# atakan-topaloglu/stable-virtual-camera

Hardware: AMD Instinct MI355X
Metric: denoising steps/sec, 1.3B Seva @ 21x576x576 views (higher is better)
Workload: dtype f16; 1 GPU; Seva 1.3B (1,263,968,004 params, random-init), one 21-view window per GPU, 576x576 px (latent 72x72), CFG batch 42, Euler-EDM step, MultiviewCFG(1.2) cfg 2.0; novel_views_per_sec = value x (T - 1 input view) / 50 steps per window; views=21, latent=72, windows=1

## Files before the change

### stable-virtual-camera_amd/csrc/attention.hip

```cpp
#include "attn_common.h"

#include <stdlib.h>

namespace {
typedef __fp16 p16x2_t __attribute__((ext_vector_type(2)));
__device__ __forceinline__ p16x2_t pack_p(float e0, float e1) {
  return __builtin_bit_cast(p16x2_t, __builtin_convertvector(f32x2{e0, e1}, half2_t));
}

struct AttnArgs : AttnBase {};

typedef short short8_t __attribute__((ext_vector_type(8)));

__device__ __forceinline__ half8_t tr_read_pair(const char* a0, const char* a1) {
  short4_t lo = __builtin_amdgcn_ds_read_tr16_b64_v4i16((__attribute__((address_space(3))) short4_t*)a0);
  short4_t hi = __builtin_amdgcn_ds_read_tr16_b64_v4i16((__attribute__((address_space(3))) short4_t*)a1);
  short8_t s = __builtin_shufflevector(lo, hi, 0, 1, 2, 3, 4, 5, 6, 7);
  return __builtin_bit_cast(half8_t, s);
}

__device__ __forceinline__ int v_chunk_swz(int row, int chunk) { return chunk ^ (((row >> 1) & 1) << 2); }

__device__ __forceinline__ float half_wave_max(float v) {
  float a = v, b = v;
  asm volatile("s_nop 1\n\tv_permlane32_swap_b32 %0, %1" : "+v"(a), "+v"(b));
  return fmaxf(a, b);
}

template <int NW, int KT, bool USE_TR, bool DBGK, bool PRE, int NBUF = 3>
__global__ __launch_bounds__(NW * 64, 3) void attn_kernel(AttnArgs p) {
  constexpr int KB = KT / 32;
  const int dbg = DBGK ? p.dbg : 0;
  static_assert(NBUF == 3 || NBUF == 1, "the three-buffer ring, or one buffer for a single tile");
  static_assert(NBUF * 2 * KT * 128 >= NW * 32 * 128, "the epilogue stages NW images of 32 rows in the K/V buffers");

  __shared__ __attribute__((aligned(16))) char smem[NBUF * 2 * KT * 128];
  constexpr int BUF_BYTES = 2 * KT * 128;
  typedef AttnRing<KT, NW, BUF_BYTES, v_chunk_swz> Ring;

  const int tid = threadIdx.x;
  const int lane = tid & 63;
  const int wave = tid >> 6;
  const int qi = lane & 31, hh = lane >> 5;

  AttnWg w;
  attn_decode<false>(p, KT, w);
  const int qb = w.qb;
  const half_t* const qbase = attn_q_base(p, w);
  const half_t* const kbase = attn_kv_base(p, w, p.k);
  const half_t* const vbase = attn_kv_base(p, w, p.v);
  half_t* const obase = attn_o_base(p, w);

  const int qrow = qb * (32 * NW) + wave * 32 + qi;
  const int qrow_c = qrow < p.lq ? qrow : p.lq - 1;

  half8_t qf[4];
#pragma unroll
  for (int s = 0; s < 4; ++s)
    qf[s] = *(const half8_t*)(qbase + (int64_t)qrow_c * p.q_sl + 16 * s + 8 * hh);

  f32x16 acc_o[2];
#pragma unroll
  for (int d = 0; d < 2; ++d)
#pragma unroll
    for (int r = 0; r < 16; ++r) acc_o[d][r] = 0.f;
  constexpr float RESCALE_THR = 8.0f;
  float m_run = PRE ? 0.f : -1e30f, l_run = 0.f;
  f32x16 neg_m[2];
#pragma unroll
  for (int r = 0; r < 16; ++r) neg_m[0][r] = neg_m[1][r] = 0.f;
  const float c = p.scale_log2;

  const int nt = (p.lk + KT - 1) / KT;
  Ring ring(kbase, vbase, p.k_sl, p.lk, smem, lane, wave);

  const int g16 = lane >> 4, i16 = lane & 15, q4 = i16 >> 2, p4 = i16 & 3;

  auto tile = [&](int buf, auto masked_c, int kt) {
    constexpr bool MASKED = decltype(masked_c)::value;
    const char* const lds_k = smem + buf * BUF_BYTES;
    const char* const lds_v = lds_k + KT * 128;
    const bool more2 = attn_ring_prefetch(kt, nt, buf, !(dbg & 1), ring);

    f32x16 sc[KB];
    __builtin_amdgcn_s_setprio(1);
#pragma unroll
    for (int kb = 0; kb < KB; ++kb) {
      const int krow = 32 * kb + qi;
      if (!(dbg & 8)) {
#pragma unroll
        for (int s = 0; s < 4; ++s) {
          const half8_t kf =
              *(const half8_t*)(lds_k + krow * 128 + (k_chunk_swz(krow, 2 * s + hh) << 4));
          if (s == 0) {
            f32x16 c0;
            if (PRE) {
              c0 = neg_m[kb & 1];
            } else {
#pragma unroll
              for (int r = 0; r < 16; ++r) c0[r] = 0.f;
            }
            sc[kb] = __builtin_amdgcn_mfma_f32_32x32x16_f16(kf, qf[s], c0, 0, 0, 0);
          } else {
            sc[kb] = __builtin_amdgcn_mfma_f32_32x32x16_f16(kf, qf[s], sc[kb], 0, 0, 0);
          }
        }
      } else {
        asm volatile("" : "=v"(sc[kb]));
      }
    }
    __builtin_amdgcn_s_setprio(0);
    if (MASKED) {
#pragma unroll
      for (int kb = 0; kb < KB; ++kb)
#pragma unroll
        for (int r = 0; r < 16; ++r) {
          const int key = kt * KT + 32 * kb + (r & 3) + 8 * (r >> 2) + 4 * hh;
          if (key >= p.lk) sc[kb][r] = -1e30f;
        }
    }
    float mx = -1e30f;
    if (!(dbg & 2)) {
      float mk[KB];
#pragma unroll
      for (int kb = 0; kb < KB; ++kb) {
        mk[kb] = sc[kb][0];
#pragma unroll
        for (int r = 1; r < 16; ++r) mk[kb] = fmaxf(mk[kb], sc[kb][r]);
      }
#pragma unroll
      for (int kb = 0; kb < KB; ++kb) mx = fmaxf(mx, mk[kb]);
      mx = half_wave_max(mx);
    }
    if (PRE) {
      const bool first = kt == 0;
      if (!(dbg & 2) && (first || __any(mx > RESCALE_THR))) {
        const float delta = first ? mx : fmaxf(mx, 0.f);
        const float alpha = first ? 1.0f : __builtin_amdgcn_exp2f(-delta);
        m_run += delta;
#pragma unroll
        for (int r = 0; r < 16; ++r) neg_m[0][r] = neg_m[1][r] = -m_run;
        asm volatile("" : "+v"(neg_m[0]), "+v"(neg_m[1]));
        l_run *= alpha;
#pragma unroll
        for (int d = 0; d < 2; ++d)
#pragma unroll
          for (int r = 0; r < 16; ++r) acc_o[d][r] *= alpha;
#pragma unroll
        for (int kb = 0; kb < KB; ++kb)
#pragma unroll
          for (int r = 0; r < 16; ++r) sc[kb][r] -= delta;
      }
    } else {
    const float mxs = mx * c;
    if (!(dbg & 2) && __any(mxs > m_run + RESCALE_THR)) {
      const float m_new = fmaxf(m_run, mxs);
      const float alpha = __builtin_amdgcn_exp2f(m_run - m_new);
      m_run = m_new;
      l_run *= alpha;
#pragma unroll
      for (int d = 0; d < 2; ++d)
#pragma unroll
        for (int r = 0; r < 16; ++r) acc_o[d][r] *= alpha;
    }
    }
    typedef __fp16 fp16x2_t __attribute__((ext_vector_type(2)));
    const fp16x2_t ones2 = {(__fp16)1.0f, (__fp16)1.0f};
    float lsum4[4] = {0.f, 0.f, 0.f, 0.f};
    half8_t pf[KB][2];
#pragma unroll
    for (int kb = 0; kb < KB; ++kb)
#pragma unroll
      for (int s2 = 0; s2 < 2; ++s2) {
        fp16x2_t pk[4];
#pragma unroll
        for (int j = 0; j < 4; ++j) {
          float e0, e1;
          if (!(dbg & 2)) {
            if (PRE) {
              e0 = __builtin_amdgcn_exp2f(sc[kb][8 * s2 + 2 * j]);
              e1 = __builtin_amdgcn_exp2f(sc[kb][8 * s2 + 2 * j + 1]);
            } else {
              e0 = __builtin_amdgcn_exp2f(__builtin_fmaf(sc[kb][8 * s2 + 2 * j], c, -m_run));
              e1 = __builtin_amdgcn_exp2f(__builtin_fmaf(sc[kb][8 * s2 + 2 * j + 1], c, -m_run));
            }
          } else {
            e0 = sc[kb][8 * s2 + 2 * j];
            e1 = sc[kb][8 * s2 + 2 * j + 1];
          }
          pk[j] = pack_p(e0, e1);
          if (!(dbg & 2)) lsum4[j] = __builtin_amdgcn_fdot2(pk[j], ones2, lsum4[j], false);
        }
        pf[kb][s2] = __builtin_bit_cast(half8_t, pk);
      }
    l_run += (lsum4[0] + lsum4[1]) + (lsum4[2] + lsum4[3]);

    __builtin_amdgcn_s_setprio(1);
#pragma unroll
    for (int db = 0; db < 2; ++db) {
#pragma unroll
      for (int kb = 0; kb < KB; ++kb) {
#pragma unroll
        for (int s2 = 0; s2 < 2; ++s2) {
          const int r0 = 32 * kb + 16 * s2 + 4 * hh;
          half8_t vf;
          if (USE_TR) {
            const int colbyte = (32 * db + 16 * (g16 & 1) + 4 * p4) * 2;
            const int ch = colbyte >> 4, within = colbyte & 15;
            const int ra = r0 + q4, rb = r0 + 8 + q4;
            vf = tr_read_pair(lds_v + ra * 128 + (v_chunk_swz(ra, ch) << 4) + within,
                              lds_v + rb * 128 + (v_chunk_swz(rb, ch) << 4) + within);
          } else {
            const int d = 32 * db + qi;
#pragma unroll
            for (int j = 0; j < 8; ++j) {
              const int row = r0 + (j & 3) + 8 * (j >> 2);
              vf[j] = *(const half_t*)(lds_v + row * 128 + (v_chunk_swz(row, d >> 3) << 4) + (d & 7) * 2);
            }
          }
          if (!(dbg & 4)) acc_o[db] = __builtin_amdgcn_mfma_f32_32x32x16_f16(vf, pf[kb][s2], acc_o[db], 0, 0, 0);
          else asm volatile("" ::"v"(vf), "v"(pf[kb][s2]));
        }
      }
    }
    __builtin_amdgcn_s_setprio(0);
    attn_ring_arrive<Ring::G>(more2);
  };
  attn_ring_start<Ring::G>(nt, ring, qf);
  const int nfull = p.lk / KT;
  int buf = 0;
  for (int kt = 0; kt < nfull; ++kt) {
    tile(buf, std::false_type{}, kt);
    buf = buf == 2 ? 0 : buf + 1;
  }
  if (nfull < nt) tile(buf, std::true_type{}, nfull);

  const float l_tot = l_run + __shfl_xor(l_run, 32, 64);
  const float inv = 1.0f / l_tot;
  __syncthreads();
  char* const ow = smem + wave * (32 * 128);
  attn_stage_o32(ow, qi, hh, acc_o, inv);
  attn_store_rows<4>(ow, obase, p.o_sl, qb * (32 * NW) + wave * 32, p.lq, lane);
}

template <int KT, bool SPLIT = false>
__global__ __launch_bounds__(256, 2) void attn2_kernel(AttnArgs p) {
  constexpr int NW = 4, QB = 2, KB = KT / 32;
  __shared__ __attribute__((aligned(16))) char smem[3 * 2 * KT * 128];
  constexpr int BUF_BYTES = 2 * KT * 128;
  typedef AttnRing<KT, NW, BUF_BYTES, v_chunk_swz> Ring;

  const int tid = threadIdx.x;
  const int lane = tid & 63;
  const int wave = tid >> 6;
  const int qi = lane & 31, hh = lane >> 5;

  AttnWg w;
  attn_decode<SPLIT>(p, KT, w);
  const int qb = w.qb, lk = w.lk;
  const half_t* const qbase = attn_q_base(p, w);
  const half_t* const kbase = attn_kv_base(p, w, p.k);
  const half_t* const vbase = attn_kv_base(p, w, p.v);
  half_t* const obase = attn_o_base(p, w);

  half8_t qf[QB][4];
#pragma unroll
  for (int c = 0; c < QB; ++c) {
    const int qrow = qb * (32 * QB * NW) + wave * (32 * QB) + 32 * c + qi;
    const int qrow_c = qrow < p.lq ? qrow : p.lq - 1;
#pragma unroll
    for (int s = 0; s < 4; ++s)
      qf[c][s] = *(const half8_t*)(qbase + (int64_t)qrow_c * p.q_sl + 16 * s + 8 * hh);
  }

  const bool active = __builtin_amdgcn_readfirstlane(qb * (32 * QB * NW) + wave * (32 * QB)) < p.lq;
  f32x16 acc_o[QB][2];
  float m_run[QB], l_run[QB];
  f32x16 neg_m[QB];
#pragma unroll
  for (int c = 0; c < QB; ++c) {
    m_run[c] = 0.f;
    l_run[c] = 0.f;
#pragma unroll
    for (int r = 0; r < 16; ++r) neg_m[c][r] = 0.f;
#pragma unroll
    for (int d = 0; d < 2; ++d)
#pragma unroll
      for (int r = 0; r < 16; ++r) acc_o[c][d][r] = 0.f;
  }
  constexpr float P_SUM_BOUND = 16384.0f;

  const int nt = (lk + KT - 1) / KT;
  Ring ring(kbase, vbase, p.k_sl, lk, smem, lane, wave);
  const int g16 = lane >> 4, i16 = lane & 15, q4 = i16 >> 2, p4 = i16 & 3;
  typedef __fp16 fp16x2_t __attribute__((ext_vector_type(2)));
  const fp16x2_t ones2 = {(__fp16)1.0f, (__fp16)1.0f};

  auto tile = [&](int buf, auto masked_c, int kt) {
    constexpr bool MASKED = decltype(masked_c)::value;
    const char* const lds_k = smem + buf * BUF_BYTES;
    const char* const lds_v = lds_k + KT * 128;
    const bool more2 = attn_ring_prefetch(kt, nt, buf, true, ring);

    if (active) {
    f32x16 sc[QB][KB];
    __builtin_amdgcn_s_setprio(1);
    if constexpr (!SPLIT) {
      half8_t kfa[KB][4];
#pragma unroll
      for (int kb = 0; kb < KB; ++kb) {
        const int krow = 32 * kb + qi;
#pragma unroll
        for (int s = 0; s < 4; ++s) kfa[kb][s] = *(const half8_t*)(lds_k + krow * 128 + (k_chunk_swz(krow, 2 * s + hh) << 4));
      }
      __builtin_amdgcn_sched_barrier(0);
#pragma unroll
      for (int kb = 0; kb < KB; ++kb)
#pragma unroll
        for (int s = 0; s < 4; ++s)
#pragma unroll
          for (int c = 0; c < QB; ++c)
            sc[c][kb] = __builtin_amdgcn_mfma_f32_32x32x16_f16(kfa[kb][s], qf[c][s], s == 0 ? neg_m[c] : sc[c][kb], 0, 0, 0);
    } else {
#pragma unroll
    for (int kb = 0; kb < KB; ++kb) {
      const int krow = 32 * kb + qi;
#pragma unroll
      for (int s = 0; s < 4; ++s) {
        const half8_t kf = *(const half8_t*)(lds_k + krow * 128 + (k_chunk_swz(krow, 2 * s + hh) << 4));
#pragma unroll
        for (int c = 0; c < QB; ++c) {
          if (s == 0) {
            sc[c][kb] = __builtin_amdgcn_mfma_f32_32x32x16_f16(kf, qf[c][s], neg_m[c], 0, 0, 0);
          } else {
            sc[c][kb] = __builtin_amdgcn_mfma_f32_32x32x16_f16(kf, qf[c][s], sc[c][kb], 0, 0, 0);
          }
        }
      }
    }
    }
    __builtin_amdgcn_s_setprio(0);
    half8_t pf[QB][KB][2];
#pragma unroll
    for (int c = 0; c < QB; ++c) {
      if (MASKED) {
#pragma unroll
        for (int kb = 0; kb < KB; ++kb)
#pragma unroll
          for (int r = 0; r < 16; ++r) {
            const int key = kt * KT + 32 * kb + (r & 3) + 8 * (r >> 2) + 4 * hh;
            if (key >= lk) sc[c][kb][r] = -1e30f;
          }
      }
      float ls[4];
      const auto exp_pack = [&]() {
        ls[0] = ls[1] = ls[2] = ls[3] = 0.f;
#pragma unroll
        for (int kb = 0; kb < KB; ++kb)
#pragma unroll
          for (int s2 = 0; s2 < 2; ++s2) {
            fp16x2_t pk[4];
#pragma unroll
            for (int j = 0; j < 4; ++j) {
              const float e0 = __builtin_amdgcn_exp2f(sc[c][kb][8 * s2 + 2 * j]);
              const float e1 = __builtin_amdgcn_exp2f(sc[c][kb][8 * s2 + 2 * j + 1]);
              pk[j] = pack_p(e0, e1);
              ls[j] = __builtin_amdgcn_fdot2(pk[j], ones2, ls[j], false);
            }
            pf[c][kb][s2] = __builtin_bit_cast(half8_t, pk);
          }
        return (ls[0] + ls[1]) + (ls[2] + ls[3]);
      };
      float tot = exp_pack();
      const bool first = kt == 0;
      if (__builtin_expect(first || __any(!(tot < P_SUM_BOUND)), 0)) {
        float mk[KB];
#pragma unroll
        for (int kb = 0; kb < KB; ++kb) {
          mk[kb] = sc[c][kb][0];
#pragma unroll
          for (int r = 1; r < 16; ++r) mk[kb] = fmaxf(mk[kb], sc[c][kb][r]);
        }
        float mx = mk[0];
#pragma unroll
        for (int kb = 1; kb < KB; ++kb) mx = fmaxf(mx, mk[kb]);
        mx = half_wave_max(mx);
        const float delta = first ? mx : fmaxf(mx, 0.f);
        const float alpha = first ? 1.0f : __builtin_amdgcn_exp2f(-delta);
        m_run[c] += delta;
        l_run[c] *= alpha;
#pragma unroll
        for (int r = 0; r < 16; ++r) neg_m[c][r] = -m_run[c];
#pragma unroll
        for (int d = 0; d < 2; ++d)
#pragma unroll
          for (int r = 0; r < 16; ++r) acc_o[c][d][r] *= alpha;
#pragma unroll
        for (int kb = 0; kb < KB; ++kb)
#pragma unroll
          for (int r = 0; r < 16; ++r) sc[c][kb][r] -= delta;
        tot = exp_pack();
      }
      l_run[c] += tot;
    }
    __builtin_amdgcn_s_setprio(1);
#pragma unroll
    for (int db = 0; db < 2; ++db)
#pragma unroll
      for (int kb = 0; kb < KB; ++kb)
#pragma unroll
        for (int s2 = 0; s2 < 2; ++s2) {
          const int r0 = 32 * kb + 16 * s2 + 4 * hh;
          const int colbyte = (32 * db + 16 * (g16 & 1) + 4 * p4) * 2;
          const int ch = colbyte >> 4, within = colbyte & 15;
          const int ra = r0 + q4, rb = r0 + 8 + q4;
          const half8_t vf = tr_read_pair(lds_v + ra * 128 + (v_chunk_swz(ra, ch) << 4) + within,
                                          lds_v + rb * 128 + (v_chunk_swz(rb, ch) << 4) + within);
#pragma unroll
          for (int c = 0; c < QB; ++c)
            acc_o[c][db] = __builtin_amdgcn_mfma_f32_32x32x16_f16(vf, pf[c][kb][s2], acc_o[c][db], 0, 0, 0);
        }
    __builtin_amdgcn_s_setprio(0);
    }
    attn_ring_arrive<Ring::G>(more2);
  };
  attn_ring_start<Ring::G>(nt, ring, qf);
  const int nfull = lk / KT;
  int buf = 0;
  for (int kt = 0; kt < nfull; ++kt) {
    tile(buf, std::false_type{}, kt);
    buf = buf == 2 ? 0 : buf + 1;
  }
  if (nfull < nt) tile(buf, std::true_type{}, nfull);

  if constexpr (SPLIT) {
    const int64_t row0 = attn_part_row0(p, w);
#pragma unroll
    for (int c = 0; c < QB; ++c) {
      const int qrow = qb * (32 * QB * NW) + wave * (32 * QB) + 32 * c + qi;
      const float l_tot = l_run[c] + __shfl_xor(l_run[c], 32, 64);
      if (qrow < p.lq) {
        float* const po = p.part_o + (row0 + qrow) * 64;
#pragma unroll
        for (int db = 0; db < 2; ++db)
#pragma unroll
          for (int t = 0; t < 4; ++t)
            *(f32x4*)(po + 32 * db + 8 * t + 4 * hh) =
                f32x4{acc_o[c][db][4 * t], acc_o[c][db][4 * t + 1], acc_o[c][db][4 * t + 2], acc_o[c][db][4 * t + 3]};
        if (hh == 0) {
          float* const pm = p.part_ml + (row0 + qrow) * 2;
          pm[0] = m_run[c];
          pm[1] = l_tot;
        }
      }
    }
    return;
  }
  __syncthreads();
  char* const ow = smem + wave * QB * (32 * 128);
#pragma unroll
  for (int c = 0; c < QB; ++c) {
    const float l_tot = l_run[c] + __shfl_xor(l_run[c], 32, 64);
    attn_stage_o32(ow + c * (32 * 128), qi, hh, acc_o[c], 1.0f / l_tot);
  }
  attn_store_rows<4 * QB>(ow, obase, p.o_sl, qb * (32 * QB * NW) + wave * (32 * QB), p.lq, lane);
}

__device__ __forceinline__ int v16_chunk_swz(int row, int chunk) { return chunk ^ (((row >> 1) & 3) << 1); }

template <int KT, bool SPLIT = false>
__global__ __launch_bounds__(256, 2) void attn16_kernel(AttnArgs p) {
  constexpr int NW = 4, NQ = 4, NKB = KT / 16, NJ = KT / 32;
  __shared__ __attribute__((aligned(16))) char smem[3 * 2 * KT * 128];
  constexpr int BUF_BYTES = 2 * KT * 128;
  typedef AttnRing<KT, NW, BUF_BYTES, v16_chunk_swz> Ring;
  static_assert(3 * BUF_BYTES >= NW * 64 * 128, "the output staging re-uses the ring");

  const int tid = threadIdx.x;
  const int lane = tid & 63;
  const int wave = tid >> 6;
  const int i16 = lane & 15, g = lane >> 4;

  AttnWg w;
  attn_decode<SPLIT>(p, KT, w);
  const int qb = w.qb, lk = w.lk;
  const half_t* const qbase = attn_q_base(p, w);
  const half_t* const kbase = attn_kv_base(p, w, p.k);
  const half_t* const vbase = attn_kv_base(p, w, p.v);
  half_t* const obase = attn_o_base(p, w);

  const int wq0 = qb * (64 * NW) + wave * 64;
  half8_t qf[NQ][2];
#pragma unroll
  for (int c = 0; c < NQ; ++c) {
    const int qrow = wq0 + 16 * c + i16;
    const int qrow_c = qrow < p.lq ? qrow : p.lq - 1;
#pragma unroll
    for (int ks = 0; ks < 2; ++ks) qf[c][ks] = *(const half8_t*)(qbase + (int64_t)qrow_c * p.q_sl + 32 * ks + 8 * g);
  }
  const bool active = __builtin_amdgcn_readfirstlane(wq0) < p.lq;
  f32x4 acc_o[NQ][4];
  float m_run[NQ], l_run[NQ];
  f32x4 neg_m[NQ];
#pragma unroll
  for (int c = 0; c < NQ; ++c) {
    m_run[c] = 0.f;
    l_run[c] = 0.f;
    neg_m[c] = f32x4{0.f, 0.f, 0.f, 0.f};
#pragma unroll
    for (int d = 0; d < 4; ++d) acc_o[c][d] = f32x4{0.f, 0.f, 0.f, 0.f};
  }
  constexpr float P_SUM_BOUND = 16384.0f;

  const int nt = (lk + KT - 1) / KT;
  Ring ring(kbase, vbase, p.k_sl, lk, smem, lane, wave);
  const int q4 = i16 >> 2, p4 = i16 & 3;
  typedef __fp16 fp16x2_t __attribute__((ext_vector_type(2)));
  const fp16x2_t ones2 = {(__fp16)1.0f, (__fp16)1.0f};

  auto tile = [&](int buf, auto masked_c, int kt) {
    constexpr bool MASKED = decltype(masked_c)::value;
    const char* const lds_k = smem + buf * BUF_BYTES;
    const char* const lds_v = lds_k + KT * 128;
    const bool more2 = attn_ring_prefetch(kt, nt, buf, true, ring);

    if (active) {
      f32x4 sc[NQ][NKB];
#pragma unroll
      for (int kb = 0; kb < NKB; ++kb) {
        const int krow = 16 * kb + i16;
#pragma unroll
        for (int ks = 0; ks < 2; ++ks) {
          const half8_t kf = *(const half8_t*)(lds_k + krow * 128 + (k_chunk_swz(krow, 4 * ks + g) << 4));
#pragma unroll
          for (int c = 0; c < NQ; ++c)
            sc[c][kb] = __builtin_amdgcn_mfma_f32_16x16x32_f16(kf, qf[c][ks], ks == 0 ? neg_m[c] : sc[c][kb], 0, 0, 0);
        }
      }
      half8_t pf[NQ][NJ];
#pragma unroll
      for (int c = 0; c < NQ; ++c) {
        if (MASKED) {
#pragma unroll
          for (int kb = 0; kb < NKB; ++kb)
#pragma unroll
            for (int r = 0; r < 4; ++r)
              if (kt * KT + 16 * kb + 4 * g + r >= lk) sc[c][kb][r] = -1e30f;
        }
        float ls[4];
        const auto exp_pack = [&]() {
          ls[0] = ls[1] = ls[2] = ls[3] = 0.f;
#pragma unroll
          for (int j = 0; j < NJ; ++j) {
            fp16x2_t pk[4];
#pragma unroll
            for (int h = 0; h < 2; ++h)
#pragma unroll
              for (int e = 0; e < 2; ++e) {
                const float e0 = __builtin_amdgcn_exp2f(sc[c][2 * j + h][2 * e]);
                const float e1 = __builtin_amdgcn_exp2f(sc[c][2 * j + h][2 * e + 1]);
                pk[2 * h + e] = pack_p(e0, e1);
                ls[2 * h + e] = __builtin_amdgcn_fdot2(pk[2 * h + e], ones2, ls[2 * h + e], false);
              }
            pf[c][j] = __builtin_bit_cast(half8_t, pk);
          }
          return (ls[0] + ls[1]) + (ls[2] + ls[3]);
        };
        float tot = exp_pack();
        const bool first = kt == 0;
        if (__builtin_expect(first || __any(!(tot < P_SUM_BOUND)), 0)) {
          float mx = sc[c][0][0];
#pragma unroll
          for (int kb = 0; kb < NKB; ++kb)
#pragma unroll
            for (int r = 0; r < 4; ++r) mx = fmaxf(mx, sc[c][kb][r]);
          mx = fmaxf(mx, __shfl_xor(mx, 16, 64));
          mx = fmaxf(mx, __shfl_xor(mx, 32, 64));
          const float delta = first ? mx : fmaxf(mx, 0.f);
          const float alpha = first ? 1.0f : __builtin_amdgcn_exp2f(-delta);
          m_run[c] += delta;
          l_run[c] *= alpha;
#pragma unroll
          for (int r = 0; r < 4; ++r) neg_m[c][r] = -m_run[c];
#pragma unroll
          for (int d = 0; d < 4; ++d)
#pragma unroll
            for (int r = 0; r < 4; ++r) acc_o[c][d][r] *= alpha;
#pragma unroll
          for (int kb = 0; kb < NKB; ++kb)
#pragma unroll
            for (int r = 0; r < 4; ++r) sc[c][kb][r] -= delta;
          tot = exp_pack();
        }
        l_run[c] += tot;
      }
      half8_t vfa[4][NJ];
#pragma unroll
      for (int db = 0; db < 4; ++db)
#pragma unroll
        for (int j = 0; j < NJ; ++j) {
          const int ra = 32 * j + 4 * g + q4, rb = ra + 16;
          const int colbyte = (16 * db + 4 * p4) * 2;
          const int ch = colbyte >> 4, within = colbyte & 15;
          vfa[db][j] = tr_read_pair(lds_v + ra * 128 + (v16_chunk_swz(ra, ch) << 4) + within,
                                    lds_v + rb * 128 + (v16_chunk_swz(rb, ch) << 4) + within);
        }
      __builtin_amdgcn_sched_barrier(0);
#pragma unroll
      for (int db = 0; db < 4; ++db)
#pragma unroll
        for (int j = 0; j < NJ; ++j)
#pragma unroll
          for (int c = 0; c < NQ; ++c) acc_o[c][db] = __builtin_amdgcn_mfma_f32_16x16x32_f16(vfa[db][j], pf[c][j], acc_o[c][db], 0, 0, 0);
    }
    attn_ring_arrive<Ring::G>(more2);
  };
  attn_ring_start<Ring::G>(nt, ring, qf);
  const int nfull = lk / KT;
  int buf = 0;
  for (int kt = 0; kt < nfull; ++kt) {
    tile(buf, std::false_type{}, kt);
    buf = buf == 2 ? 0 : buf + 1;
  }
  if (nfull < nt) tile(buf, std::true_type{}, nfull);

  float l_tot[NQ];
#pragma unroll
  for (int c = 0; c < NQ; ++c) {
    float l = l_run[c];
    l += __shfl_xor(l, 16, 64);
    l += __shfl_xor(l, 32, 64);
    l_tot[c] = l;
  }
  if constexpr (SPLIT) {
    attn_write_partial16(p, w, wq0, acc_o, m_run, l_tot, i16, g);
    return;
  }
  attn_store_o16(smem, obase, p.o_sl, wq0, p.lq, acc_o, l_tot, lane, wave, i16, g);
}

__global__ __launch_bounds__(256) void attn_combine_kernel(AttnArgs p, int64_t rows_all) {
  const int64_t i = (int64_t)blockIdx.x * 256 + threadIdx.x;
  if (i >= rows_all * 8) return;
  const int64_t row = i >> 3;
  const int ch = (int)(i & 7);
  float m[4], l[4], mx = -3.0e38f;
#pragma unroll
  for (int s = 0; s < 4; ++s)
    if (s < p.nsplit) {
      const float* pm = p.part_ml + ((int64_t)s * rows_all + row) * 2;
      m[s] = pm[0];
      l[s] = pm[1];
      mx = fmaxf(mx, m[s]);
    }
  float o[8] = {0.f, 0.f, 0.f, 0.f, 0.f, 0.f, 0.f, 0.f}, lt = 0.f;
#pragma unroll
  for (int s = 0; s < 4; ++s)
    if (s < p.nsplit) {
      const float w = __builtin_amdgcn_exp2f(m[s] - mx);
      lt += w * l[s];
      const float* po = p.part_o + ((int64_t)s * rows_all + row) * 64 + 8 * ch;
      const f32x4 a = first_read(*(const f32x4*)po), b = first_read(*(const f32x4*)(po + 4));
#pragma unroll
      for (int r = 0; r < 4; ++r) {
        o[r] += w * a[r];
        o[4 + r] += w * b[r];
      }
    }
  const float inv = 1.0f / lt;
  half8_t h;
#pragma unroll
  for (int r = 0; r < 8; ++r) h[r] = (half_t)(o[r] * inv);
  const int64_t q = row % p.lq, bh = row / p.lq;
  const int head = (int)(bh % p.heads);
  const int64_t batch = bh / p.heads;
  const int64_t b0 = batch / p.nb1, b1 = batch - b0 * p.nb1;
  *(half8_t*)(p.out + b0 * p.o_sb0 + b1 * p.o_sb1 + head * 64 + q * p.o_sl + 8 * ch) = h;
}


template <int NW, int KT, int NBUF = 3>
int launch(const AttnArgs& a, int64_t batch, hipStream_t s, bool use_tr, bool pre) {
  AttnArgs args = a;
  args.qblocks = (a.lq + 32 * NW - 1) / (32 * NW);
  SEVA_REQUIRE(NBUF == 3 || a.lk <= KT, "attention: the one-buffer kernel takes one K/V tile (lk=%d > %d)", a.lk, KT);
  const int64_t nb = batch * a.heads * args.qblocks;
  if (int rc = attn_check_grid("attention", nb)) return rc;
  const dim3 grid((unsigned)nb), block(NW * 64);
  if (args.dbg && !pre)
    hipLaunchKernelGGL((attn_kernel<NW, KT, true, true, false, NBUF>), grid, block, 0, s, args);
  else if (!use_tr)
    hipLaunchKernelGGL((attn_kernel<NW, KT, false, false, false, NBUF>), grid, block, 0, s, args);
  else if (pre)
    hipLaunchKernelGGL((attn_kernel<NW, KT, true, false, true, NBUF>), grid, block, 0, s, args);
  else
    hipLaunchKernelGGL((attn_kernel<NW, KT, true, false, false, NBUF>), grid, block, 0, s, args);
  return seva_check_launch("attn_kernel");
}

constexpr bool kAttnShort2Default = false;

}

int seva_attn_combine_launch(const float* part_o, const float* part_ml, int nsplit, void* out, int64_t o_sb0, int64_t o_sb1,
                             int64_t o_sl, int nb1, int heads, int lq, int64_t rows_all, hipStream_t s) {
  AttnArgs a{};
  a.out = (half_t*)out;
  a.o_sb0 = o_sb0; a.o_sb1 = o_sb1; a.o_sl = o_sl;
  a.nb1 = nb1; a.heads = heads; a.lq = lq;
  a.part_o = (float*)part_o; a.part_ml = (float*)part_ml; a.nsplit = nsplit;
  hipLaunchKernelGGL(attn_combine_kernel, dim3((unsigned)((rows_all * 8 + 255) / 256)), dim3(256), 0, s, a, rows_all);
  return seva_check_launch("attn_combine_kernel");
}

extern "C" int seva_attention_f16(const seva_attn_desc* d, seva_stream_t stream) {
  if (int rc = attn_check_desc(d, "attention", true)) return rc;
  if (int rc = attn_check_ptrs("attention", {d->q, d->k, d->v, d->out})) return rc;
  AttnArgs a{};
  attn_fill_base(a, d);
  a.v = (const half_t*)d->v;
  a.scale_log2 = d->scale * 1.44269504088896340736f;
  a.dbg = g_seva_knobs.attn_dbg > 0 ? g_seva_knobs.attn_dbg : 0;
  const int64_t batch = (int64_t)d->nb0 * d->nb1;
  const bool use_tr = g_seva_knobs.attn_no_tr != 1;
  hipStream_t s = (hipStream_t)stream;
  const double flops = 4.0 * (double)batch * d->heads * (double)d->lq * (double)d->lk * 64.0;
  const double alg_bytes = (double)batch * d->heads * 64.0 * 2.0 * (2.0 * (double)d->lq + 2.0 * (double)d->lk);
  SevaProfScope prof(2, flops, s, alg_bytes);
  const bool pre = d->q_prescaled != 0;
  SEVA_REQUIRE(!pre || use_tr, "attention: q_prescaled is not available on the SEVA_ATTN_NO_TR debug path");
  if (d->lq <= 32) return launch<1, 32>(a, batch, s, use_tr, pre);
  if (d->lq <= 64 && d->lk <= 64 && (g_seva_knobs.attn_short2 < 0 ? kAttnShort2Default : g_seva_knobs.attn_short2 == 1))
    return launch<2, 64, 1>(a, batch, s, use_tr, pre);
  const int two = g_seva_knobs.attn_two;
  if (pre && use_tr && !a.dbg && ((two < 0 && d->lq >= SEVA_ATTN_LONG_MIN_LQ) || ((two == 1 || two == 2 || two == 4) && d->lq >= 512))) {
    const bool k16 = two == 4 || two < 0;
    const int qrows = 256;
    AttnArgs args = a;
    args.qblocks = (a.lq + qrows - 1) / qrows;
    const int64_t nb = batch * a.heads * args.qblocks;
    if (int rc = attn_check_grid("attention", nb)) return rc;
    int nsplit = d->lk >= SEVA_ATTN_SPLIT_MIN_LK ? 2 : 1;
    if (g_seva_knobs.attn_split >= 0) nsplit = g_seva_knobs.attn_split > 4 ? 4 : g_seva_knobs.attn_split;
    const int nt_all = (d->lk + 63) / 64;
    while (nsplit >= 2 && (nt_all + nsplit - 1) / nsplit * (nsplit - 1) >= nt_all) --nsplit;
    if (nsplit >= 2 && d->split_ws != nullptr) {
      const int64_t rows_all = batch * a.heads * (int64_t)a.lq;
      if (int rc = attn_split_setup(args, d, "attention", nsplit, rows_all, nb)) return rc;
      if (k16) hipLaunchKernelGGL((attn16_kernel<64, true>), dim3((unsigned)(nb * nsplit)), dim3(256), 0, s, args);
      else hipLaunchKernelGGL((attn2_kernel<64, true>), dim3((unsigned)(nb * nsplit)), dim3(256), 0, s, args);
      int rc = seva_check_launch("attn16_kernel / attn2_kernel <split>");
      if (rc) return rc;
      hipLaunchKernelGGL(attn_combine_kernel, dim3((unsigned)((rows_all * 8 + 255) / 256)), dim3(256), 0, s, args, rows_all);
      return seva_check_launch("attn_combine_kernel");
    }
    if (k16) hipLaunchKernelGGL((attn16_kernel<64>), dim3((unsigned)nb), dim3(256), 0, s, args);
    else hipLaunchKernelGGL((attn2_kernel<64>), dim3((unsigned)nb), dim3(256), 0, s, args);
    return seva_check_launch("attn16_kernel / attn2_kernel");
  }
  return launch<4, 64>(a, batch, s, use_tr, pre);
}
```

Before: 11.04 denoising steps/s.

## Compute softmax row sums with MFMA and specialize first tile in flash attention

Replaces per-lane fdot2 row-sum accumulation with an MFMA against a ones matrix, which yields the full cross-lane row sum directly and drops the final shuffle reduction. The first key tile gets its own compile-time specialized path. On the overflow path, scores are recomputed from LDS so the rescale check is hoisted out of the per-head-chunk loop and checked once across all chunks. This adds extra MFMA work per tile and a rarely taken recompute in exchange for fewer VALU ops and less branching in the softmax.

After: 11.22 denoising steps/s (median of 6 runs). +1.7%, better.

```diff
diff --git a/stable-virtual-camera_amd/csrc/attention.hip b/stable-virtual-camera_amd/csrc/attention.hip
--- a/stable-virtual-camera_amd/csrc/attention.hip
+++ b/stable-virtual-camera_amd/csrc/attention.hip
@@ -516,10 +516,13 @@
   Ring ring(kbase, vbase, p.k_sl, lk, smem, lane, wave);
   const int q4 = i16 >> 2, p4 = i16 & 3;
   typedef __fp16 fp16x2_t __attribute__((ext_vector_type(2)));
-  const fp16x2_t ones2 = {(__fp16)1.0f, (__fp16)1.0f};
-
-  auto tile = [&](int buf, auto masked_c, int kt) {
+  half8_t ones8;
+#pragma unroll
+  for (int r = 0; r < 8; ++r) ones8[r] = (half_t)1.0f;
+
+  auto tile = [&](int buf, auto masked_c, auto first_c, int kt) {
     constexpr bool MASKED = decltype(masked_c)::value;
+    constexpr bool FIRST = decltype(first_c)::value;
     const char* const lds_k = smem + buf * BUF_BYTES;
     const char* const lds_v = lds_k + KT * 128;
     const bool more2 = attn_ring_prefetch(kt, nt, buf, true, ring);
@@ -538,62 +541,95 @@
         }
       }
       half8_t pf[NQ][NJ];
-#pragma unroll
-      for (int c = 0; c < NQ; ++c) {
-        if (MASKED) {
-#pragma unroll
-          for (int kb = 0; kb < NKB; ++kb)
-#pragma unroll
-            for (int r = 0; r < 4; ++r)
-              if (kt * KT + 16 * kb + 4 * g + r >= lk) sc[c][kb][r] = -1e30f;
-        }
-        float ls[4];
-        const auto exp_pack = [&]() {
-          ls[0] = ls[1] = ls[2] = ls[3] = 0.f;
-#pragma unroll
-          for (int j = 0; j < NJ; ++j) {
-            fp16x2_t pk[4];
-#pragma unroll
-            for (int h = 0; h < 2; ++h)
-#pragma unroll
-              for (int e = 0; e < 2; ++e) {
-                const float e0 = __builtin_amdgcn_exp2f(sc[c][2 * j + h][2 * e]);
-                const float e1 = __builtin_amdgcn_exp2f(sc[c][2 * j + h][2 * e + 1]);
-                pk[2 * h + e] = pack_p(e0, e1);
-                ls[2 * h + e] = __builtin_amdgcn_fdot2(pk[2 * h + e], ones2, ls[2 * h + e], false);
+      const auto mask_tail = [&](f32x4 (&s)[NKB]) {
+#pragma unroll
+        for (int kb = 0; kb < NKB; ++kb)
+#pragma unroll
+          for (int r = 0; r < 4; ++r)
+            if (kt * KT + 16 * kb + 4 * g + r >= lk) s[kb][r] = -1e30f;
+      };
+      const auto exp_pack = [&](int c, const f32x4 (&s)[NKB]) {
+        f32x4 tl = f32x4{0.f, 0.f, 0.f, 0.f};
+#pragma unroll
+        for (int j = 0; j < NJ; ++j) {
+          fp16x2_t pk[4];
+#pragma unroll
+          for (int h = 0; h < 2; ++h)
+#pragma unroll
+            for (int e = 0; e < 2; ++e) {
+              const float e0 = __builtin_amdgcn_exp2f(s[2 * j + h][2 * e]);
+              const float e1 = __builtin_amdgcn_exp2f(s[2 * j + h][2 * e + 1]);
+              pk[2 * h + e] = pack_p(e0, e1);
+            }
+          pf[c][j] = __builtin_bit_cast(half8_t, pk);
+          tl = __builtin_amdgcn_mfma_f32_16x16x32_f16(ones8, pf[c][j], tl, 0, 0, 0);
+        }
+        return tl[0];
+      };
+      const auto new_reference = [&](int c, f32x4 (&s)[NKB], bool need) {
+        float mx = s[0][0];
+#pragma unroll
+        for (int kb = 0; kb < NKB; ++kb)
+#pragma unroll
+          for (int r = 0; r < 4; ++r) mx = fmaxf(mx, s[kb][r]);
+        mx = fmaxf(mx, __shfl_xor(mx, 16, 64));
+        mx = fmaxf(mx, __shfl_xor(mx, 32, 64));
+        const float delta = FIRST ? mx : need ? fmaxf(mx, 0.f) : 0.f;
+        m_run[c] += delta;
+#pragma unroll
+        for (int r = 0; r < 4; ++r) neg_m[c][r] = -m_run[c];
+        if (!FIRST) {
+          const float alpha = __builtin_amdgcn_exp2f(-delta);
+          l_run[c] *= alpha;
+#pragma unroll
+          for (int d = 0; d < 4; ++d)
+#pragma unroll
+            for (int r = 0; r < 4; ++r) acc_o[c][d][r] *= alpha;
+        }
+#pragma unroll
+        for (int kb = 0; kb < NKB; ++kb)
+#pragma unroll
+          for (int r = 0; r < 4; ++r) s[kb][r] -= delta;
+        return exp_pack(c, s);
+      };
+      float tot[NQ];
+      if (FIRST) {
+#pragma unroll
+        for (int c = 0; c < NQ; ++c) {
+          if (MASKED) mask_tail(sc[c]);
+          tot[c] = new_reference(c, sc[c], true);
+        }
+      } else {
+        bool over = false;
+#pragma unroll
+        for (int c = 0; c < NQ; ++c) {
+          if (MASKED) mask_tail(sc[c]);
+          tot[c] = exp_pack(c, sc[c]);
+          if (c > 0) over |= !(tot[c - 1] < P_SUM_BOUND);
+          __builtin_amdgcn_sched_barrier(0);
+        }
+        over |= !(tot[NQ - 1] < P_SUM_BOUND);
+        if (__builtin_expect(__any(over), 0)) {
+#pragma unroll
+          for (int c = 0; c < NQ; ++c) {
+            const bool need = __any(!(tot[c] < P_SUM_BOUND));
+            f32x4 s1[NKB];
+#pragma unroll
+            for (int kb = 0; kb < NKB; ++kb) {
+              const int krow = 16 * kb + i16;
+#pragma unroll
+              for (int ks = 0; ks < 2; ++ks) {
+                const half8_t kf = *(const half8_t*)(lds_k + krow * 128 + (k_chunk_swz(krow, 4 * ks + g) << 4));
+                s1[kb] = __builtin_amdgcn_mfma_f32_16x16x32_f16(kf, qf[c][ks], ks == 0 ? neg_m[c] : s1[kb], 0, 0, 0);
               }
-            pf[c][j] = __builtin_bit_cast(half8_t, pk);
+            }
+            if (MASKED) mask_tail(s1);
+            tot[c] = new_reference(c, s1, need);
           }
-          return (ls[0] + ls[1]) + (ls[2] + ls[3]);
-        };
-        float tot = exp_pack();
-        const bool first = kt == 0;
-        if (__builtin_expect(first || __any(!(tot < P_SUM_BOUND)), 0)) {
-          float mx = sc[c][0][0];
-#pragma unroll
-          for (int kb = 0; kb < NKB; ++kb)
-#pragma unroll
-            for (int r = 0; r < 4; ++r) mx = fmaxf(mx, sc[c][kb][r]);
-          mx = fmaxf(mx, __shfl_xor(mx, 16, 64));
-          mx = fmaxf(mx, __shfl_xor(mx, 32, 64));
-          const float delta = first ? mx : fmaxf(mx, 0.f);
-          const float alpha = first ? 1.0f : __builtin_amdgcn_exp2f(-delta);
-          m_run[c] += delta;
-          l_run[c] *= alpha;
-#pragma unroll
-          for (int r = 0; r < 4; ++r) neg_m[c][r] = -m_run[c];
-#pragma unroll
-          for (int d = 0; d < 4; ++d)
-#pragma unroll
-            for (int r = 0; r < 4; ++r) acc_o[c][d][r] *= alpha;
-#pragma unroll
-          for (int kb = 0; kb < NKB; ++kb)
-#pragma unroll
-            for (int r = 0; r < 4; ++r) sc[c][kb][r] -= delta;
-          tot = exp_pack();
-        }
-        l_run[c] += tot;
-      }
+        }
+      }
+#pragma unroll
+      for (int c = 0; c < NQ; ++c) l_run[c] += tot[c];
       half8_t vfa[4][NJ];
 #pragma unroll
       for (int db = 0; db < 4; ++db)
@@ -617,21 +653,18 @@
   };
   attn_ring_start<Ring::G>(nt, ring, qf);
   const int nfull = lk / KT;
-  int buf = 0;
-  for (int kt = 0; kt < nfull; ++kt) {
-    tile(buf, std::false_type{}, kt);
+  if (nfull > 0) tile(0, std::false_type{}, std::true_type{}, 0);
+  else tile(0, std::true_type{}, std::true_type{}, 0);
+  int buf = 1;
+  for (int kt = 1; kt < nfull; ++kt) {
+    tile(buf, std::false_type{}, std::false_type{}, kt);
     buf = buf == 2 ? 0 : buf + 1;
   }
-  if (nfull < nt) tile(buf, std::true_type{}, nfull);
+  if (nfull > 0 && nfull < nt) tile(buf, std::true_type{}, std::false_type{}, nfull);
 
   float l_tot[NQ];
 #pragma unroll
-  for (int c = 0; c < NQ; ++c) {
-    float l = l_run[c];
-    l += __shfl_xor(l, 16, 64);
-    l += __shfl_xor(l, 32, 64);
-    l_tot[c] = l;
-  }
+  for (int c = 0; c < NQ; ++c) l_tot[c] = l_run[c];
   if constexpr (SPLIT) {
     attn_write_partial16(p, w, wq0, acc_o, m_run, l_tot, i16, g);
     return;
```
